# bbw7561135/Compton2d

Hardware: AMD Instinct MI355X
Metric: photon-packet-steps/sec (whole node) at 1/2/4/8 GPUs; % HBM roofline (higher is better)
Workload: dtype f64

## Files before the change

### compton2d_amd/csrc/c2d_device.hpp

```cpp
#ifndef C2D_DEVICE_HPP
#define C2D_DEVICE_HPP

#include <stdint.h>
#include "../../include/compton2d.h"

namespace c2d {

#define C2D_IDX_BUCKETS 2048
struct Geo {
  double z[C2D_MAXZONE + 1];
  double r[C2D_MAXZONE + 1];
  double E_ph[C2D_N_VOL + 1];
  double E_field[C2D_NPHFIELD + 1];
  double hu[C2D_NPHOMAX + 2];
  double Elcmin[C2D_NPHLCMAX + 1];
  double Elcmax[C2D_NPHLCMAX + 1];
  double mu[C2D_NMUMAX + 1];
  int16_t eph_start[C2D_IDX_BUCKETS];
  int16_t efl_start[C2D_IDX_BUCKETS];
  int32_t eph_k0, efl_k0;
};
constexpr int GEO_DOUBLES = (int)(sizeof(Geo) / sizeof(double));

struct SpecDev {
// ... 155 lines not shown
  const double* f_nt;
  const double* Pnt;
  const double* n_e;
  const double* vfrac;
  const double* ewsv;
  const int64_t* vol_prefix;
  const int64_t* surf_prefix;
  const double* surf_ew;
  const double* surf_tbb;
  const int32_t* surf_spec;
  const double* tbbl;
  const SpecDev* spectra;
  int32_t n_spectra, nslot;
  const double* comtab;
  double comtab_du_inv;
  double egg_min;
  CensusSoA cin, cout;
  int64_t n_cin, cap_cout;
  uint32_t cens_chunk;
  unsigned long long* n_cout;
  const int32_t* clist;
  const int32_t* pool;
  const unsigned long long* pool_n;
  unsigned long long* pool_head;
  int32_t* out_list;
  unsigned long long* n_out;
  int32_t* relist;
  unsigned long long* n_relist;
  unsigned long long* relist_head;
  int64_t* cstate;
  double* ev;
  int64_t cap_ev;
  unsigned long long* n_ev_sh;
  int64_t cap_ev_sh;
  int64_t cap_q;
  PktSoA pk;
  int64_t cap_pk;
  int64_t n_cens_items, n_vol_items, n_surf_items;
  int64_t vol_cens_base;
  int64_t n_vol_global, n_surf_global;
  double* T;
  double* nf_rep;
  TallyOff off;
  unsigned long long* cnt;
  int32_t* err;
  int32_t lds_cells;
  int32_t evq_cap;
  unsigned long long* prof;
  const uint16_t* cdf_guide;
  int32_t cr_sent;
  const double* refl_E;
  const double* refl_P;
  const double* refl_W;
  double* refl_out;
};
#define C2D_CDF_GUIDE 256

#define C2D_KN_CAP_DEFAULT 32
#define C2D_SC_K1_DEFAULT 16
struct GenArgs {
  const ScatRec* q2_in;
  const ScatRec* q3_in;
  ScatRec* q2_out;
  ScatRec* q3_out;
  unsigned long long* n2_out;
  unsigned long long* n3_out;
  unsigned long long* n_pk;
  unsigned long long* work_counter;
  unsigned long long* work_sh;
  unsigned long long* n_hard;
  int64_t* hard;
  int64_t item_begin, item_end;
  int64_t n_items;
  int64_t n2_in, n3_in;
  int32_t gen;
  int32_t kn_cap;
  int32_t sc_k1;
};

enum : int32_t {
  VZ_TEA = 0, VZ_TNA, VZ_NE, VZ_B, VZ_FPAIR, VZ_ZSURF, VZ_VOL, VZ_EP, VZ_LMIN, VZ_N = 12
};
enum : int32_t { VO_B = 0, VO_ESY, VO_ECY, VO_ETH, VO_ETOT, VO_N = 8 };
struct VemParams {
  const double* zin;
  const double* f_nt;
  const double* gnt;
  const double* E_ph;
  const double* mcd;
  double dE, pow3_15, dt;
  double* kappa;
  double* eps_tot;
  double* eps_th;
  double* zout;
};

enum : int32_t {
  FZ_VOL = 0, FZ_TEA, FZ_TNA, FZ_NE, FZ_B, FZ_ELSY, FZ_ECENS, FZ_ECOLD, FZ_TURB, FZ_FPAIR,
  FZ_PNTH, FZ_N = 16
};
enum : int32_t { FO_TE = 0, FO_NE, FO_GMIN, FO_GMAX, FO_AMXWL, FO_PNTH, FO_DIAG = 8, FO_N = 16 };
enum : int32_t { FPERR_STEPS = 1, FPERR_GUARD = 2, FPERR_NF_IN = 4, FPERR_NF_OUT = 8 };

#define C2D_FP_MCD_N 16384
#define C2D_FPF_MT_Q 1024
#define C2D_FPF_MT_LO (-17)
#define C2D_FPF_MT_HI 3
#define C2D_FPF_MT_N ((C2D_FPF_MT_HI - C2D_FPF_MT_LO) * C2D_FPF_MT_Q + 1)
#define C2D_FPF_MT_K 7
#define C2D_FPF_MT_W (4 + 2 * C2D_FPF_MT_K + 24)

struct FpParams {
  int32_t nz, nr, pick_sw, inj_switch, inj_dis, g2var_switch, cf_sentinel, pair_sw;
  double time, dt, df_implicit, df_T, r_esc, r_acc;
  double r_flare, z_flare, t_flare, sigma_r, sigma_z, sigma_t, flare_amp;
  double inj_g1, inj_g2, inj_p, inj_t, inj_L, pick_rate, inj_gg, inj_sigma, inj_v;
  const Geo* geo;
  const double* gnt;
  const double* FT;
  const double* mcd;
  const double* zin;
  const double* f_in;
  const double* P_in;
  const double* nf;
  const double* ecens;
  double* f_out;
  double* P_out;
  double* zout;
  int32_t* err;
  unsigned long long* gb_key;
  double* gb_val;
  uint32_t gb_mask;
  const int32_t* zorder;
  int32_t* zq;
  int32_t ncell;
  const double* mom;
  int32_t mt_glob;
  int32_t probe;
};

struct ObsDev {
  double gam_bulk, rmax, t_offset;
  int32_t mode, n_t, n_mu, n_e;
  const double* t0; const double* t1;
  const double* mu0; const double* mu1;
  const double* E0; const double* E1;
  double* F;
  double* F2;
  double* cnt;
  int32_t lds_rows;
  int32_t sorted_t, sorted_mu, sorted_e;
};

constexpr int OBS_SET_MAX = 8;
constexpr int OBS_SET_LDS = 64 * 1024;
constexpr int OBS_SET_LDS_STATIC = 1024;

struct ObsSetMember {
  double gam_bulk, rmax, t_offset;
  double* F; double* F2; double* cnt;
  int32_t mode, n_t, n_mu, n_e;
  int32_t lds_rows;
  int32_t sorted_t, sorted_mu, sorted_e;
  int32_t edge_off, hist_off;
};

struct ObsSetDev {
  const double* edges;
  int32_t n, n_edges, n_hist;
  ObsSetMember m[OBS_SET_MAX];
};

}

#endif
```

### compton2d_amd/csrc/capi.cpp

```cpp
#include <hip/hip_runtime.h>
#include <rccl/rccl.h>

#include <algorithm>
#include <cfloat>
#include <cmath>
#include <cstdarg>
#include <cstdio>
#include <cstring>
#include <string>
#include <vector>

#include "../../include/compton2d.h"
#include "c2d_device.hpp"
#include "c2d_math.h"
#include "c2d_rng.h"
#include "pspt_host.h"
#include "plcm_host.h"
#include "reflect_host.h"
#include "c2d_censfmt.h"
#include "c2d_censtext.hpp"
#include "c2d_evparse.hpp"
#include "c2d_evtext.hpp"

using namespace c2d;
// ... 141 lines not shown
  int64_t last_compact_moved = 0;
  c2d_tally_layout L;
  Geo* geo = nullptr;
  double *gnt = nullptr, *kappa_cur = nullptr, *kappa_prev = nullptr, *eps_tot = nullptr,
         *eps_th = nullptr, *f_nt = nullptr, *Pnt = nullptr, *n_e = nullptr, *vfrac = nullptr,
         *ewsv = nullptr, *surf_ew = nullptr, *surf_tbb = nullptr, *tbbl = nullptr;
  int64_t *vol_prefix = nullptr, *surf_prefix = nullptr;
  int32_t* surf_spec = nullptr;
  SpecDev* spectra = nullptr;
  std::vector<double*> spec_bufs;
  int n_spectra = 0;
  double* comtab = nullptr;
  double* comS = nullptr;
  DevCensus cens[2];
  int cur = 0;
  int64_t n_census = 0;
  double* ev = nullptr;
  int64_t n_ev = 0;
  int64_t ev_cnt[C2D_EV_SHARDS] = {};
  bool ev_stepped = false;
  c2d_evt_writer* evt = nullptr;
  c2d_evt_times evt_times = {};
  c2d_evt_reader* evr = nullptr;
  c2d_evr_times evr_times = {};
  c2d_cens_file* cfile = nullptr;
  c2d_cens_times cens_times = {};
  unsigned long long* cens_bad = nullptr;
  hipEvent_t cens_ev[2] = {nullptr, nullptr};
  hipStream_t obs_stream = nullptr;
  hipEvent_t ev_obs_src = nullptr, ev_obs_a = nullptr, ev_obs_b = nullptr;
  bool obs_inflight = false;
  int64_t ev_cap_sh = 0;
  ScatRec *q2[2] = {nullptr, nullptr}, *q3[2] = {nullptr, nullptr};
  DevPk pk;
  double* T = nullptr;
  double* T_own = nullptr;
  double* nf_rep = nullptr;
  unsigned long long* ctl = nullptr;
  int32_t* derr = nullptr;
  KParams* dP = nullptr;
  KParams P;
  bool have_step = false;
  bool have_electrons = false;
  bool have_vem = false;
  int32_t* mono_flag = nullptr;
  double* refl_tab = nullptr;
  double* refl_out = nullptr;
  double* refl_red = nullptr;
  bool refl_stepped = false;
  ncclComm_t comm = nullptr;
  int comm_rank = 0, comm_world = 1;
  int64_t n_vol_global = 0, n_surf_global = 0;
  int eps_linear = 0;
  uint16_t* cdf_guide = nullptr;
  bool cdf_guide_on = false;
  std::vector<double> h_stage;
  double last_g0_ms = 0.0, last_all_ms = 0.0;
  float last_src_ms = 0.f;
  unsigned long long last_prof[C2D_TR_PROF_WORDS] = {};
  int64_t last_g0_steps = 0;
  double egg_min = 0.0;
  int64_t last_g0_paths = 0, last_all_paths = 0;
  int last_launches = 0;
  bool fp_ready = false;
  c2d_fp_config fpc;
  double *fp_FT = nullptr, *fp_mcd = nullptr, *fp_zin = nullptr, *fp_fin = nullptr, *fp_Pin = nullptr,
         *fp_nf = nullptr, *fp_fout = nullptr, *fp_Pout = nullptr, *fp_zout = nullptr;
  int32_t* fp_err = nullptr;
  unsigned long long* fp_gb_key = nullptr;
  double* fp_gb_val = nullptr;
  int32_t fp_mode = C2D_FP_EXACT;
  unsigned long long* fpf_gb_key = nullptr;
  double* fpf_gb_val = nullptr;
  FpParams* fp_dP = nullptr;
  int32_t* fpf_zq = nullptr;
  double* fpf_mom = nullptr;
  std::vector<int32_t> fpf_order;
  bool fpf_ordered = false;
  bool fp_auto_known = false, fp_auto_exact = false;
  int32_t last_fp_mode = -1;
  float last_fp_ms = 0.f;
  int last_fp_waves = 0;
  double *vem_zin = nullptr, *vem_fnt = nullptr, *vem_eph = nullptr, *vem_kap = nullptr,
         *vem_et = nullptr, *vem_eh = nullptr, *vem_zout = nullptr;
  float last_vem_ms = 0.f;
  bool obs_ready = false;
  ObsDev obs;
  double *obs_edges = nullptr, *obs_hist = nullptr, *obs_ev = nullptr;
  double* pspt_red = nullptr;
  c2d_pspt_deck pspt;
  bool pspt_on = false;
  int64_t obs_ev_cap = 0;
  int obs_wg_per_cu = 1;
  double obs_ms = 0.0;
  ObsSetDev oset = {};
  std::vector<ObsSetHost> oset_h;
  double* oset_edges = nullptr;
  bool oset_started = false;
  bool obs_inflight_set = false;
  int oset_wg_per_cu = 1;
  int32_t oset_launches = 0;
  double oset_ms = 0.0;
};

static int fail(c2d_ctx* c, int code, const char* fmt, ...) {
  char buf[512];
  va_list ap;
  va_start(ap, fmt);
  vsnprintf(buf, sizeof buf, fmt, ap);
  va_end(ap);
  if (c) c->err = buf;
  return code;
}

#define HIPCHK(c, x)                                                                   \
  do {                                                                                 \
    hipError_t e_ = (x);                                                               \
    if (e_ != hipSuccess)                                                              \
      return fail((c), C2D_E_HIP, "%s:%d %s: %s", __FILE__, __LINE__, #x,              \
                  hipGetErrorString(e_));                                              \
  } while (0)

template <class T>
static hipError_t dalloc(T** p, size_t n) {
  if (n == 0) n = 1;
  return hipMalloc((void**)p, n * sizeof(T));
}

extern "C" const char* c2d_version(void) { return "compton2d_amd 0.1.0 (gfx950)"; }

extern "C" const char* c2d_last_error(c2d_ctx* ctx) { return ctx ? ctx->err.c_str() : "null context"; }

static __host__ __device__ int grid_bin_host(const double* E, int n, double x) {
  int lo = 1, hi = n;
  while (lo < hi) {
    const int mid = (lo + hi) >> 1;
    if (x < E[mid + 1]) hi = mid;
    else lo = mid + 1;
  }
  return lo;
}
static void build_lookup(const double* E, int n, int16_t* start, int32_t* k0) {
  uint64_t u;
  std::memcpy(&u, &E[1], sizeof u);
  *k0 = (int32_t)(u >> 48);
  for (int b = 0; b < C2D_IDX_BUCKETS; b++) {
    const uint64_t k = (uint64_t)(*k0 + b);
    double x = 0.0;
    if (k < 0x7ff0) {
      const uint64_t v = k << 48;
      std::memcpy(&x, &v, sizeof x);
      start[b] = (int16_t)grid_bin_host(E, n, x);
    } else {
      start[b] = (int16_t)(b > 0 ? start[b - 1] : 1);
    }
  }
}

extern "C" int c2d_init(const c2d_config* cfg, c2d_ctx** out) {
  if (!cfg || !out) return C2D_E_ARG;
  *out = nullptr;
  if (cfg->nz < 1 || cfg->nr < 1 || cfg->nz > C2D_MAXZONE || cfg->nr > C2D_MAXZONE)
    return C2D_E_ARG;
  if (cfg->nphtotal < 1 || cfg->nphtotal > C2D_NPHOMAX || cfg->nph_lc < 0 ||
      cfg->nph_lc > C2D_NPHLCMAX || cfg->nmu < 1 || cfg->nmu > C2D_NMUMAX)
    return C2D_E_ARG;
  if (cfg->cr_sent < 0 || cfg->cr_sent > 4) return C2D_E_ARG;
// ... 139 lines not shown
  {
    auto aocc = cfg->comtot_mode == C2D_COMTOT_TABLE ? c2d_aux_occupancy_fast : c2d_aux_occupancy_exact;
    int bs = 0, bc = 0;
    orc = aocc(0, &bs);
    if (!orc) orc = aocc(1, &bc);
    if (orc) return fail(c, C2D_E_HIP, "occupancy query: %s", hipGetErrorString((hipError_t)orc));
    c->src_grid = c->n_cu * std::max(1, bs);
    c->sc_grid = c->n_cu * std::max(1, bc);
  }
  {
    const int64_t ccap = std::max<int64_t>(cfg->census_capacity, 1);
    c->n_ws = (int64_t)std::max(c->bundle_grid, c->max_grid) * (C2D_TR_BLOCK / 64);
    HIPCHK(c, dalloc(&c->cstate, 2 * (size_t)c->n_ws));
    HIPCHK(c, hipMemset(c->cstate, 0xff, 2 * sizeof(int64_t) * c->n_ws));
    c->chunked = cfg->census_inplace ? 1 : 0;
    if (c->chunked) {
      c->cens_chunk = C2D_CCHUNK;
      int64_t slack = 4 * c->n_ws + 64;
      if (const char* e = getenv("C2D_CHUNK_SLACK")) slack = std::max<long long>(0, atoll(e));
      c->nchunks = (ccap + C2D_CCHUNK - 1) / C2D_CCHUNK + (ccap / 16 + C2D_CCHUNK - 1) / C2D_CCHUNK + slack;
      c->cens_phys = c->nchunks * C2D_CCHUNK;
      for (int b = 0; b < 2; b++) HIPCHK(c, dalloc(&c->clist[b], (size_t)c->nchunks));
      HIPCHK(c, dalloc(&c->pool, (size_t)c->nchunks));
      HIPCHK(c, dalloc(&c->out_list, (size_t)c->nchunks));
      HIPCHK(c, dalloc(&c->relist, (size_t)c->nchunks));
      HIPCHK(c, dalloc(&c->cflag, (size_t)c->nchunks));
      HIPCHK(c, dalloc(&c->part_id, (size_t)c->n_ws));
      HIPCHK(c, dalloc(&c->part_off, (size_t)c->n_ws + 1));
    } else {
      int64_t ch = 1024;
      while (ch > 64 && ch * c->n_ws * 8 > ccap) ch >>= 1;
      c->cens_chunk = (uint32_t)ch;
      c->cens_phys = ccap + c->n_ws * ch + 64;
      c->cscan_cap = std::min<int64_t>(int64_t(1) << 27, std::max<int64_t>(int64_t(1) << 16, ccap / 16));
      if (const char* e = getenv("C2D_COMPACT_LIST")) c->cscan_cap = std::max<long long>(1, atoll(e));
      HIPCHK(c, dalloc(&c->cscan, 2 * (size_t)c->cscan_cap));
    }
    for (int b = 0; b < (c->chunked ? 1 : 2); b++) {
      for (int f = 0; f < 3; f++) HIPCHK(c, dalloc(&c->cens[b].d[f], (size_t)c->cens_phys));
      HIPCHK(c, dalloc(&c->cens[b].tg, (size_t)c->cens_phys));
    }
  }
  HIPCHK(c, hipStreamSynchronize(c->stream));
  return C2D_OK;
}

extern "C" void c2d_finalize(c2d_ctx* c) {
  if (!c) return;
  (void)hipSetDevice(c->cfg.device);
  if (c->stream) (void)hipStreamSynchronize(c->stream);
  if (c->obs_stream) (void)hipStreamSynchronize(c->obs_stream);
  if (c->mono_flag) (void)hipFree(c->mono_flag);
  c2d_evtext_free(c->evt);
  c2d_evparse_free(c->evr);
  c2d_censtext_free(c->cfile);
  if (c->cens_bad) (void)hipFree(c->cens_bad);
  for (hipEvent_t e : c->cens_ev)
    if (e) (void)hipEventDestroy(e);
  if (c->comm) (void)ncclCommDestroy(c->comm);
  void* ptrs[] = {c->geo, c->gnt, c->kappa_cur, c->kappa_prev, c->eps_tot, c->eps_th, c->f_nt,
                  c->Pnt, c->n_e, c->vfrac, c->ewsv, c->surf_ew, c->surf_tbb, c->tbbl,
                  c->vol_prefix, c->surf_prefix, c->surf_spec, c->spectra, c->comtab, c->comS,
                  c->ev, c->q2[0], c->q2[1], c->q3[0], c->q3[1], c->T_own, c->nf_rep, c->ctl, c->derr, c->dP,
                  c->cscan, c->ctile_cnt, c->ctile_off, c->ctile_flag, c->cstate, c->clist[0], c->clist[1],
                  c->pool, c->out_list, c->relist, c->cflag, c->part_id, c->part_off, c->tmp_rec};
  for (void* p : ptrs)
    if (p) (void)hipFree(p);
  for (int b = 0; b < 2; b++) {
    for (int f = 0; f < 3; f++)
      if (c->cens[b].d[f]) (void)hipFree(c->cens[b].d[f]);
    if (c->cens[b].tg) (void)hipFree(c->cens[b].tg);
  }
  for (double* p : c->spec_bufs) (void)hipFree(p);
  void* rptrs[] = {c->refl_tab, c->refl_out, c->refl_red};
  for (void* p : rptrs)
    if (p) (void)hipFree(p);
  void* optrs[] = {c->obs_edges, c->obs_hist, c->obs_ev, c->pspt_red, c->cdf_guide, c->oset_edges};
  for (void* p : optrs)
    if (p) (void)hipFree(p);
  for (ObsSetHost& m : c->oset_h) {
    if (m.hist) (void)hipFree(m.hist);
    if (m.red) (void)hipFree(m.red);
  }
  void* vptrs[] = {c->vem_zin, c->vem_fnt, c->vem_eph, c->vem_kap, c->vem_et, c->vem_eh, c->vem_zout};
  for (void* q : vptrs)
    if (q) (void)hipFree(q);
  void* fptrs[] = {c->fp_FT, c->fp_mcd, c->fp_zin, c->fp_fin, c->fp_Pin, c->fp_nf, c->fp_fout, c->fp_Pout,
                   c->fp_zout, c->fp_err, c->fp_gb_key, c->fp_gb_val, c->fpf_gb_key, c->fpf_gb_val,
                   c->fp_dP, c->fpf_zq, c->fpf_mom};
  for (void* p : fptrs)
    if (p) (void)hipFree(p);
  c->pk.release();
  if (c->ev_g0a) (void)hipEventDestroy(c->ev_g0a);
  if (c->ev_g0b) (void)hipEventDestroy(c->ev_g0b);
  if (c->ev_g0t) (void)hipEventDestroy(c->ev_g0t);
  if (c->ev_end) (void)hipEventDestroy(c->ev_end);
  if (c->obs_stream) (void)hipStreamSynchronize(c->obs_stream);
  if (c->ev_obs_src) (void)hipEventDestroy(c->ev_obs_src);
  if (c->ev_obs_a) (void)hipEventDestroy(c->ev_obs_a);
  if (c->ev_obs_b) (void)hipEventDestroy(c->ev_obs_b);
  if (c->obs_stream) (void)hipStreamDestroy(c->obs_stream);
  if (c->stream) (void)hipStreamDestroy(c->stream);
  delete c;
}

static void gather3(const c2d_ctx* c, const c2d_array3& a, int n, double* out) {
  for (int j = 0; j < c->nz; j++)
    for (int k = 0; k < c->nr; k++) {
      double* o = out + (size_t)(j * c->nr + k) * n;
      if (!a.data) {
        std::fill(o, o + n, 0.0);
        continue;
      }
      const double* base = a.data + j * a.s_j + k * a.s_k;
      if (a.s_i == 1)
        memcpy(o, base, sizeof(double) * n);
      else
        for (int i = 0; i < n; i++) o[i] = base[i * a.s_i];
    }
}
static double at2(const c2d_array2& a, int j, int k) {
  return a.data ? a.data[j * a.s_j + k * a.s_k] : 0.0;
}

extern "C" int c2d_set_clock(c2d_ctx* c, int32_t ncycle, double time, double dt) {
  if (!c) return C2D_E_ARG;
  c->P.ncycle = ncycle;
  c->P.time = time;
  c->P.dt = dt;
  c->P.cdt = 2.9979245620e10 * dt;
  c->P.cens_wlim = c->cfg.trk_variant == C2D_TRK_2012_11 ? 1.0 : 0.99999999;
  c->P.step_key = c2d_step_key(c->cfg.seed, ncycle);
  return C2D_OK;
}

__global__ void __launch_bounds__(256) c2d_check_monotone(const double* __restrict__ a, int rows, int n,
                                                          int32_t* __restrict__ flag) {
  for (int64_t t = blockIdx.x * (int64_t)blockDim.x + threadIdx.x; t < (int64_t)rows * n;
       t += (int64_t)gridDim.x * blockDim.x) {
    const int i = (int)(t % n);
    if (i > 0 && !(a[t] >= a[t - 1])) atomicOr(flag, 1);
  }
}

__global__ void __launch_bounds__(256) c2d_check_finite(const double* __restrict__ a, int64_t n, int32_t bit,
                                                        int32_t* __restrict__ flag) {
  bool bad = false;
  for (int64_t t = blockIdx.x * (int64_t)blockDim.x + threadIdx.x; t < n; t += (int64_t)gridDim.x * blockDim.x)
    bad |= !(fabs(a[t]) <= DBL_MAX);
  if (bad) atomicOr(flag, bit);
}

static void check_finite(c2d_ctx* c, const double* a, int64_t n, int32_t bit, int32_t* flag, hipStream_t st) {
  if (n <= 0) return;
  const int grid = (int)std::max<int64_t>(1, std::min<int64_t>((n + 255) / 256, (int64_t)c->n_cu * 4));
  hipLaunchKernelGGL(c2d_check_finite, dim3(grid), dim3(256), 0, st, a, n, bit, flag);
}

static bool all_finite(const double* a, size_t n) {
  for (size_t i = 0; i < n; i++)
    if (!std::isfinite(a[i])) return false;
  return true;
}

__global__ void __launch_bounds__(256) c2d_cdf_guide(const double* __restrict__ eps_tot,
                                                     const double* __restrict__ eps_th, int ncell, int n,
                                                     uint16_t* __restrict__ guide) {
// ... 1707 lines not shown
      const double* dg = zo + FO_DIAG;
      double* p;
      if ((p = m2(out->Te_new, j, k))) *p = zo[FO_TE];
      if (dg[C2D_FP_SKIPPED] == 0.0) {
        for (int i = 0; i < C2D_NUM_NT && !el_dev; i++) {
          out->f_nt.data[i * out->f_nt.s_i + j * out->f_nt.s_j + k * out->f_nt.s_k] =
              fout[(size_t)cell * C2D_NUM_NT + i];
          out->Pnt.data[i * out->Pnt.s_i + j * out->Pnt.s_j + k * out->Pnt.s_k] =
              pout[(size_t)cell * C2D_NUM_NT + i];
        }
        if ((p = m2(out->n_e, j, k))) *p = zo[FO_NE];
        if ((p = m2(out->gmin, j, k))) *p = zo[FO_GMIN];
        if ((p = m2(out->gmax, j, k))) *p = zo[FO_GMAX];
        if ((p = m2(out->amxwl, j, k))) *p = zo[FO_AMXWL];
        if ((p = m2(out->p_nth, j, k))) *p = zo[FO_PNTH];
        E_old = E_old + dg[C2D_FP_E_OLD];
        E_new = E_new + dg[C2D_FP_E_NEW];
        hr = hr + dg[C2D_FP_HR];
        hr_st = hr_st + dg[C2D_FP_HR_ST];
        if (dg[C2D_FP_DELTA_T] > dT_max) dT_max = dg[C2D_FP_DELTA_T];
      }
      if ((p = m2(out->tea, j, k)) && a2(in->tna, j, k, 0.0) > 1.) {
        double t = zo[FO_TE];
        t = (1.0e3 < t) ? 1.0e3 : t;
        t = (5.0 > t) ? 5.0 : t;
        *p = t;
      }
      if (out->zone_diag)
        memcpy(out->zone_diag + (size_t)cell * C2D_FP_NDIAG, dg, sizeof(double) * C2D_FP_NDIAG);
    }
  out->E_tot_old = E_old;
  out->E_tot_new = E_new;
  out->hr_total = hr;
  out->hr_st_total = hr_st;
  out->dT_max = dT_max;
  return C2D_OK;
}

extern "C" int c2d_electron_state(c2d_ctx* c, c2d_marray3 f_nt, c2d_marray3 Pnt) {
  if (!c) return C2D_E_ARG;
  if (!c->have_electrons) return fail(c, C2D_E_STATE, "c2d_electron_state: no electron state yet");
  HIPCHK(c, hipSetDevice(c->cfg.device));
  const size_t nnt = (size_t)c->ncell * C2D_NUM_NT;
  std::vector<double> h(nnt);
  const c2d_marray3* views[2] = {&f_nt, &Pnt};
  const double* src[2] = {c->f_nt, c->Pnt};
  for (int v = 0; v < 2; v++) {
    const c2d_marray3& m = *views[v];
    if (!m.data) continue;
    HIPCHK(c, hipMemcpy(h.data(), src[v], nnt * sizeof(double), hipMemcpyDeviceToHost));
    for (int j = 0; j < c->nz; j++)
      for (int k = 0; k < c->nr; k++)
        for (int i = 0; i < C2D_NUM_NT; i++)
          m.data[i * m.s_i + j * m.s_j + k * m.s_k] = h[((size_t)j * c->nr + k) * C2D_NUM_NT + i];
  }
  return C2D_OK;
}

extern "C" int c2d_last_fp_ms(c2d_ctx* c, double* ms) {
  if (!c || !ms) return C2D_E_ARG;
  *ms = c->last_fp_ms;
  return C2D_OK;
}

extern "C" int c2d_volume_em(c2d_ctx* c, const c2d_vem_in* in, c2d_vem_out* out) {
  if (!c || !in || !out) return C2D_E_ARG;
  if (!in->tea.data || !in->tna.data || !in->n_e.data || !in->B_field.data || !in->f_pair.data ||
      !in->zsurf.data || !in->vol.data)
    return fail(c, C2D_E_ARG, "c2d_volume_em: missing input array");
  const bool el_dev = !in->f_nt.data;
  if (el_dev && !c->have_electrons)
    return fail(c, C2D_E_STATE, "c2d_volume_em: f_nt NULL but no electron state on the device");
  HIPCHK(c, hipSetDevice(c->cfg.device));
  const int nz = c->nz, nr = c->nr;
  const size_t nc = (size_t)c->ncell;
  if (!c->vem_zin) {
    HIPCHK(c, dalloc(&c->vem_zin, nc * VZ_N));
    HIPCHK(c, dalloc(&c->vem_fnt, nc * C2D_NUM_NT));
    HIPCHK(c, dalloc(&c->vem_eph, (size_t)C2D_N_VOL));
    HIPCHK(c, dalloc(&c->vem_kap, nc * C2D_N_VOL));
    HIPCHK(c, dalloc(&c->vem_et, nc * C2D_N_VOL));
    HIPCHK(c, dalloc(&c->vem_eh, nc * C2D_N_VOL));
    HIPCHK(c, dalloc(&c->vem_zout, nc * VO_N));
  }
  if (int rc = ensure_mcd(c)) return rc;
  const double dE = c2d_exp(c2d_log(1.0e20) / (double)C2D_N_VOL);
  std::vector<double> eph(C2D_N_VOL);
  double E = 1.0e-10 / dE;
  for (int i = 0; i < C2D_N_VOL; i++) {
    E = E * dE;
    eph[i] = E;
  }
  std::vector<double> zin(nc * VZ_N, 0.0), fnt(nc * C2D_NUM_NT);
  for (int j = 0; j < nz; j++)
    for (int k = 0; k < nr; k++) {
      const size_t cell = (size_t)j * nr + k;
      double* z = &zin[cell * VZ_N];
      z[VZ_TEA] = at2(in->tea, j, k);
      z[VZ_TNA] = at2(in->tna, j, k);
      z[VZ_NE] = at2(in->n_e, j, k);
      z[VZ_B] = at2(in->B_field, j, k);
      z[VZ_FPAIR] = at2(in->f_pair, j, k);
      if (c->cfg.pair_switch == 1 && !(z[VZ_FPAIR] < 1.0e-10))
        return fail(c, C2D_E_ARG,
                    "volume_em: pair annihilation (pair_switch=1, f_pair=%g in zone (%d,%d)) needs "
                    "a positron population; positrons are inert here (H6)", z[VZ_FPAIR], j + 1, k + 1);
      z[VZ_ZSURF] = at2(in->zsurf, j, k);
      z[VZ_VOL] = at2(in->vol, j, k);
      z[VZ_EP] = in->ep_switch.data ? (double)in->ep_switch.data[j * in->ep_switch.s_j + k * in->ep_switch.s_k] : 0.0;
      const double dz = (j == 0) ? c->cfg.z[0] : c->cfg.z[j] - c->cfg.z[j - 1];
      const double drr = (k == 0) ? c->cfg.r[0] - c->cfg.rmin : c->cfg.r[k] - c->cfg.r[k - 1];
      z[VZ_LMIN] = (dz < drr) ? dz : drr;
      for (int i = 0; i < C2D_NUM_NT && !el_dev; i++)
        fnt[cell * C2D_NUM_NT + i] = in->f_nt.data[i * in->f_nt.s_i + j * in->f_nt.s_j + k * in->f_nt.s_k];
    }
  if (!all_finite(zin.data(), zin.size()) || !all_finite(fnt.data(), el_dev ? 0 : fnt.size()))
    return fail(c, C2D_E_NONFINITE, "c2d_volume_em: NaN/Inf in the zone inputs or f_nt");
  c->have_vem = false;
  const hipStream_t st = c->stream;
  HIPCHK(c, hipMemcpyAsync(c->vem_zin, zin.data(), zin.size() * sizeof(double), hipMemcpyHostToDevice, st));
  if (!el_dev)
    HIPCHK(c, hipMemcpyAsync(c->vem_fnt, fnt.data(), fnt.size() * sizeof(double), hipMemcpyHostToDevice, st));
  HIPCHK(c, hipMemcpyAsync(c->vem_eph, eph.data(), eph.size() * sizeof(double), hipMemcpyHostToDevice, st));
  VemParams P;
  P.zin = c->vem_zin; P.f_nt = el_dev ? c->f_nt : c->vem_fnt; P.gnt = c->gnt; P.E_ph = c->vem_eph; P.mcd = c->fp_mcd;
  P.dE = dE; P.pow3_15 = c2d_pow(3.0, 1.5); P.dt = in->dt;
  P.kappa = c->vem_kap; P.eps_tot = c->vem_et; P.eps_th = c->vem_eh; P.zout = c->vem_zout;
  HIPCHK(c, hipEventRecord(c->ev_g0a, st));
  int rc = c2d_launch_vem(&P, (int)nc, st);
  if (rc) return fail(c, C2D_E_HIP, "vem launch: %s", hipGetErrorString((hipError_t)rc));
  HIPCHK(c, hipEventRecord(c->ev_g0b, st));
  if (!c->mono_flag) HIPCHK(c, dalloc(&c->mono_flag, 1));
  HIPCHK(c, hipMemsetAsync(c->mono_flag, 0, sizeof(int32_t), st));
  if (el_dev) check_finite(c, c->f_nt, (int64_t)nc * C2D_NUM_NT, 1, c->mono_flag, st);
  check_finite(c, c->vem_kap, (int64_t)nc * C2D_N_VOL, 2, c->mono_flag, st);
  check_finite(c, c->vem_et, (int64_t)nc * C2D_N_VOL, 2, c->mono_flag, st);
  check_finite(c, c->vem_eh, (int64_t)nc * C2D_N_VOL, 2, c->mono_flag, st);
  HIPCHK(c, hipGetLastError());
  int32_t vflag = 0;
  HIPCHK(c, hipMemcpyAsync(&vflag, c->mono_flag, sizeof vflag, hipMemcpyDeviceToHost, st));
  std::vector<double> kap(out->kappa_tot.data ? nc * C2D_N_VOL : 0),
      et(out->eps_tot.data ? nc * C2D_N_VOL : 0), eh(out->eps_th.data ? nc * C2D_N_VOL : 0), zo(nc * VO_N);
  if (!kap.empty())
    HIPCHK(c, hipMemcpyAsync(kap.data(), c->vem_kap, kap.size() * sizeof(double), hipMemcpyDeviceToHost, st));
  if (!et.empty())
    HIPCHK(c, hipMemcpyAsync(et.data(), c->vem_et, et.size() * sizeof(double), hipMemcpyDeviceToHost, st));
  if (!eh.empty())
    HIPCHK(c, hipMemcpyAsync(eh.data(), c->vem_eh, eh.size() * sizeof(double), hipMemcpyDeviceToHost, st));
  HIPCHK(c, hipMemcpyAsync(zo.data(), c->vem_zout, zo.size() * sizeof(double), hipMemcpyDeviceToHost, st));
  HIPCHK(c, hipStreamSynchronize(st));
  (void)hipEventElapsedTime(&c->last_vem_ms, c->ev_g0a, c->ev_g0b);
  if (vflag & 1) return fail(c, C2D_E_NONFINITE, "c2d_volume_em: NaN/Inf in the device f_nt");
  bool zo_ok = true;
  for (size_t cell = 0; cell < nc; cell++) zo_ok = zo_ok && all_finite(&zo[cell * VO_N], VO_ETOT + 1);
  if ((vflag & 2) || !zo_ok)
    return fail(c, C2D_E_NONFINITE, "c2d_volume_em: NaN/Inf in the emission/absorption tables or "
                "Eloss outputs (volume2d.f:343-390)");
  c->have_vem = true;
  if (out->E_ph) std::copy(eph.begin(), eph.end(), out->E_ph);
  auto put3 = [&](c2d_marray3& m, const std::vector<double>& v, size_t cell, int j, int k) {
    if (!m.data) return;
    for (int i = 0; i < C2D_N_VOL; i++)
      m.data[i * m.s_i + j * m.s_j + k * m.s_k] = v[cell * C2D_N_VOL + i];
  };
  auto put2 = [&](c2d_marray2& m, int j, int k, double v) {
    if (m.data) m.data[j * m.s_j + k * m.s_k] = v;
  };
  for (int j = 0; j < nz; j++)
    for (int k = 0; k < nr; k++) {
      const size_t cell = (size_t)j * nr + k;
      put3(out->kappa_tot, kap, cell, j, k);
      put3(out->eps_tot, et, cell, j, k);
      put3(out->eps_th, eh, cell, j, k);
      const double* o = &zo[cell * VO_N];
      put2(out->B_field, j, k, o[VO_B]);
      put2(out->Eloss_sy, j, k, o[VO_ESY]);
      put2(out->Eloss_cy, j, k, o[VO_ECY]);
      put2(out->Eloss_th, j, k, o[VO_ETH]);
      put2(out->Eloss_tot, j, k, o[VO_ETOT]);
    }
  return C2D_OK;
}

extern "C" int c2d_last_vem_ms(c2d_ctx* c, double* ms) {
  if (!c || !ms) return C2D_E_ARG;
  *ms = c->last_vem_ms;
  return C2D_OK;
}

static int obs_settle(c2d_ctx* c);

extern "C" int c2d_obs_begin(c2d_ctx* c, const c2d_obs_bins* b) {
  if (!c || !b) return C2D_E_ARG;
  if ((b->mode != C2D_OBS_SED && b->mode != C2D_OBS_LC) || b->n_t < 1 || b->n_t > C2D_OBS_MAX_T ||
      b->n_mu < 1 || b->n_mu > C2D_OBS_MAX_MU || b->n_e < 1 || b->n_e > C2D_OBS_MAX_E ||
      !b->t0 || !b->t1 || !b->mu0 || !b->mu1 || !b->E0 || !b->E1 || !(b->gam_bulk >= 1.0))
    return fail(c, C2D_E_ARG, "c2d_obs_begin: bad binning");
  if (b->mode == C2D_OBS_SED && b->n_mu != 1)
    return fail(c, C2D_E_ARG, "c2d_obs_begin: the SED mode has one angular window");
  c->pspt_on = false;
  c->obs_ready = false;
  HIPCHK(c, hipSetDevice(c->cfg.device));
  { const int rc = obs_settle(c); if (rc) return rc; }
  if (c->obs_edges) (void)hipFree(c->obs_edges);
  if (c->obs_hist) (void)hipFree(c->obs_hist);
  c->obs_edges = c->obs_hist = nullptr;
  const int ne = 2 * (b->n_t + b->n_mu + b->n_e);
  std::vector<double> h;
  h.reserve(ne);
  h.insert(h.end(), b->t0, b->t0 + b->n_t);
// ... 909 lines not shown
```

### compton2d_amd/csrc/vem.hip

```cpp
#include <hip/hip_runtime.h>
#include <stdint.h>

#include "c2d_device.hpp"
#include "c2d_math.h"
#include "c2d_wave.hpp"

namespace c2d {
namespace {

using namespace wave;
constexpr int VEM_BLOCK = 448;
constexpr int NT = C2D_NUM_NT;
constexpr int NV = C2D_N_VOL;
constexpr double PI_REF = 3.1415926536;
constexpr double C_LIGHT = 2.9979245620e10;

__device__ __forceinline__ double expk13(double t) {
  const double c1 = F32(0.35502805), c2 = F32(0.25881940);
  if (t <= 1.0) {
    double z3 = 1.5 * t;
    const double zs = c2d_pow(z3, 0.3333333333333333);
    const double z = zs * zs;
    z3 = z3 * z3;
    const double f1 = 1.0 + z3 / 6.0 * (1.0 + z3 / 30.0 * (1.0 + z3 / 56.0));
    const double f2 = z * (1.0 + z3 / 12.0 * (1.0 + z3 / 42.0 * (1.0 + z3 / 90.0)));
    return c2d_exp_bf(t) * PI_REF * 1.7320508 / zs * (c1 * f1 - c2 * f2);
  }
  const double z = 1.0 / (72.0 * t);
  const double poly = 1.0 - 5.0 * z * (1.0 - 38.5 * z);
  return __builtin_sqrt(0.5 * PI_REF / t) * poly / (1.0 + 1.0 / (1.0 + 58.0 * t * t));
}

__device__ __forceinline__ double expk43(double t) {
  if (t <= 1.0) {
    const double poly = 1.0 + t * (0.9757317 - 7.6790616e-2 * t);
    return 0.44648975 * c2d_pow(2.0 / t, 1.333333333) * poly;
  }
  const double z = 1.0 / (72.0 * t);
  const double poly = 1.0 + 55.0 * z * (1.0 - 8.5 * z);
  return __builtin_sqrt(0.5 * PI_REF / t) * poly * (1.0 + 1.0 / (1.0 + 50.0 * t * t));
}

}

__global__ void __launch_bounds__(VEM_BLOCK) c2d_vem_kernel(const VemParams P) {
  __shared__ double s_gnt[NT], s_f[NT], s_q[NT], s_gamp[NT], s_facg[NT], s_dg[NT];
  __shared__ double s_cP[NV], s_cC[NV], s_cT[NV], s_P[NV], s_Pth[NV];
  __shared__ double s_sc[8];
  __shared__ double s_mcd[4 * FPB];
  const int cell = blockIdx.x;
  const int tid = threadIdx.x, lane = tid & 63, wv = tid >> 6;
  const double* zin = P.zin + (int64_t)cell * VZ_N;
  const double tea = zin[VZ_TEA], ne = zin[VZ_NE];
  for (int i = tid; i < NT; i += VEM_BLOCK) {
    s_gnt[i] = P.gnt[i];
    s_f[i] = P.f_nt[(int64_t)cell * NT + i];
  }
  __syncthreads();
  if (wv == 0) {
    long long guard = 0;
    double B = zin[VZ_B];
    const int ep = (int)zin[VZ_EP];
    if (ep == 1 || ep == 2) {
      const double Th = (ep == 1) ? 1.957e-3 * tea : 1.066e-6 * zin[VZ_TNA];
      double uB;
      if (Th < 1.0e-2) {
        uB = 1.5 * Th + 7.5 * (Th * Th);
      } else {
        double K2b, K3b;
        mcdonald23_w(1.0 / Th, lane, P.mcd, K2b, K3b, guard, s_mcd);
        uB = K3b / K2b - Th - 1.0;
      }
      if (ep == 1)
        uB = uB * ne * 8.176e-7 * (1. + 2.0 * zin[VZ_FPAIR]);
      else
        uB = uB * ne * 1.5e-3;
      B = __builtin_sqrt(2.513e1 * uB);
    }
    const double Theta = tea / 5.11e2;
    double K2 = 0.0, K2m = 0.0, K3m = 0.0;
    const bool big = !(Theta < F32(0.2)) || !(Theta < 2.0e-1);
    if (big) mcdonald23_w(1. / Theta, lane, P.mcd, K2m, K3m, guard, s_mcd);
    if (Theta < 2.0e-1)
      K2 = 1.2533 * __builtin_sqrt(Theta) *
           (1. + 1.875 * Theta + 8.2031e-1 * (Theta * Theta) - 2.03e-1 * (Theta * Theta * Theta)) /
           c2d_exp_bf(Theta);
    else
      K2 = K2m;
    double g_av;
    if (Theta < F32(0.2)) {
      g_av = (1. + F32(4.375) * Theta + F32(7.383) * (Theta * Theta) +
              F32(3.384) * (Theta * Theta * Theta)) /
                 (1. + F32(1.875) * Theta + F32(.8203) * (Theta * Theta)) -
             Theta;
    } else {
      g_av = K3m / K2m - Theta;
    }
    if (g_av < 1.0) g_av = 1.0;
    const double gamma_R = 2.1e-3 * __builtin_sqrt(ne) / (B * __builtin_sqrt(g_av));
    const double y = gamma_R / g_av;
    const double f_rz = (y < 1.0e2) ? c2d_exp_bf(-y) : 0.;
    const double s1 = seq_sum(0.0, 0, NT - 2, lane, [&](int i) {
      const double g1 = s_gnt[i] + 1.0;
      return (g1 * g1 - 1.0) * s_f[i] * (s_gnt[i + 1] - s_gnt[i]);
    });
    if (lane == 0) {
      s_sc[0] = B; s_sc[1] = K2; s_sc[2] = f_rz; s_sc[7] = s1;
    }
  }
  __syncthreads();
  const double B = s_sc[0], K2 = s_sc[1], f_rz = s_sc[2];
  const double em = 9.109e-28, ee = 4.803e-10, sigmaT = 6.6524616e-25;
  const double nu_b = ee * B / (2 * PI_REF * em * C_LIGHT);
  for (int i = tid; i < NT; i += VEM_BLOCK) {
    const double g0 = s_gnt[i] + 1.0;
    const double gp = g0 * __builtin_sqrt(g0 * g0 - 1.0);
    s_gamp[i] = gp;
    s_q[i] = s_f[i] / gp;
    s_facg[i] = 3.0 * (g0 * g0) * nu_b;
    s_dg[i] = (i < NT - 1) ? s_gnt[i + 1] - s_gnt[i] : 0.0;
  }
  __syncthreads();
  if (tid < NV) {
    const int i = tid;
    const double Ub = (B * B) / (8.0 * PI_REF);
    const double face = P.pow3_15 * sigmaT * C_LIGHT * Ub / (PI_REF * nu_b);
    const double dE = P.dE, E = P.E_ph[i];
    const double Theta = tea / 5.11e2;
    const double kappa_C = 6.65e-25 * ne;
    const double nu_c = 2.8e6 * B, nu_min = 5.0 * nu_c, nu_p = 9.0e3 * __builtin_sqrt(ne);
    const double nu = 2.41487e17 * E;
    double j_sy = 0., kappa_sy = 0., j_cy = 0.;
    if (!(nu <= nu_p)) {
      double sum = 0., sum_k = 0.;
      for (int i2 = 0; i2 < NT - 1; i2++) {
        const double tt = nu / s_facg[i2];
        double es = 0.0;
        if (tt < 1.0e4) {
          const double eq43 = expk43(tt), eq13 = expk13(tt);
          const double ff = tt * tt * (eq43 * eq13 - F32(0.6) * tt * (eq43 - eq13) * (eq43 + eq13));
          es = face * ff * c2d_exp_bf(-2.0 * tt);
        }
        const double sd = s_f[i2] * es;
        const double sd_k = s_gamp[i2] * es;
        sum = sum + s_dg[i2] * sd;
        sum_k = sum_k + (s_q[i2] - s_q[i2 + 1]) * sd_k;
      }
      j_sy = sum * ne / (4.0 * PI_REF);
      kappa_sy = sum_k * ne / (8.0 * PI_REF * em * (nu * nu));
      if (kappa_sy < 0.) kappa_sy = -1.0 * kappa_sy;
      double f_m = 1.0;
      for (int m = 1; m <= 5; m++) {
        const double mm = (double)m;
        f_m = f_m / (4. * mm);
        const double nu_m = mm * nu_c;
        const double E_m = 4.14e-18 * nu_m;
        const double D_m = 7.07e-1 * Theta * E_m;
        const double q = (E - E_m) / D_m;
        const double x = q * q;
        if (x < 50.) {
          const double f_cy = f_rz * c2d_exp_bf(-x) * ne * (B * B) * c2d_pow(Theta, mm - 1.5) *
                              (mm + 1.0) * f_m * c2d_pow(mm, 2.0 * mm + 1.0);
          j_cy = j_cy + 8.46e-14 * f_cy * (E * E) / (E_m * E_m * E_m);
        }
      }
      if (nu > nu_min) {
        const double v = nu / (nu_c * (Theta * Theta));
        const double y = 4.5 * v;
        if (y < 1.0e6)
          j_cy = j_cy + 4.652e-12 * ne * nu /
                            (K2 * c2d_pow(v, 1.6666667e-1) * c2d_exp_bf(c2d_pow(y, 3.33333e-1)));
      }
    }
    P.kappa[(int64_t)cell * NV + i] = kappa_sy;
    const double lm = zin[VZ_LMIN];
    const double thr = (1.0 / lm > 1.0e1 * kappa_C) ? 1.0 / lm : 1.0e1 * kappa_C;
    double cP = 0.0, cC = 0.0, cT = 0.0;
    if (kappa_sy < thr) {
      cP = j_sy * E * (dE - 1.0);
      cC = j_cy * E * (dE - 1.0);
    } else {
      const double x = E / tea;
      const double tau_tot = kappa_sy * lm;
      double j_th = (x < 1.0e2) ? 1.47e-47 * (nu * nu * nu) / (c2d_exp_bf(x) - 1.0) : 1.0e-50;
      if (tau_tot < 5.0e1) j_th = j_th * (1.0 - c2d_exp_bf(-tau_tot));
      cT = j_th * E * (dE - 1.0);
    }
    s_cP[i] = cP; s_cC[i] = cC; s_cT[i] = cT;
  }
  __syncthreads();
  if (wv == 0) {
    double aP = 0.0, aT = 0.0, aC = 0.0;
    for (int c0 = 0; c0 < NV; c0 += FPB) {
      const int i = c0 + lane;
      const double vP = (i < NV) ? s_cP[i] : 0.0, vT = (i < NV) ? s_cT[i] : 0.0;
      const double vC = (i < NV) ? s_cC[i] : 0.0;
      const int mn = (NV - c0) < FPB ? (NV - c0) : FPB;
      double mP = 0.0, mT = 0.0;
      for (int m = 0; m < mn; m++) {
        aP = aP + rl(vP, m);
        aT = aT + rl(vT, m);
        aC = aC + rl(vC, m);
        if (lane == m) { mP = aP; mT = aT; }
      }
      if (i < NV) { s_P[i] = mP; s_Pth[i] = mT; }
    }
    if (lane == 0) {
      s_sc[3] = aP; s_sc[4] = aT; s_sc[5] = aC;
    }
  }
  __syncthreads();
  if (tid < NV) {
    const double P_sum = s_sc[3], sum_th = s_sc[4];
    P.eps_tot[(int64_t)cell * NV + tid] = (P_sum > 1.0e-50) ? s_P[tid] / P_sum : 0.;
    P.eps_th[(int64_t)cell * NV + tid] = (sum_th > 1.0e-50) ? s_Pth[tid] / sum_th : 0.;
  }
  if (tid == 0) {
    const double vol = zin[VZ_VOL], zs = zin[VZ_ZSURF], dt = P.dt;
    double* o = P.zout + (int64_t)cell * VO_N;
    const double esy = 1.058e-15 * ne * dt * (B * B) * s_sc[7] * vol;
    o[VO_B] = B;
    o[VO_ESY] = esy;
    o[VO_ECY] = dt * vol * s_sc[5];
    o[VO_ETH] = dt * zs * s_sc[4];
    o[VO_ETOT] = esy;
  }
}

}

extern "C" int c2d_launch_vem(const c2d::VemParams* P, int ncell, hipStream_t stream) {
  if (ncell <= 0) return 0;
  hipLaunchKernelGGL(c2d::c2d_vem_kernel, dim3(ncell), dim3(c2d::VEM_BLOCK), 0, stream, *P);
  return (int)hipGetLastError();
}
```

Measured before the change: 291.7 billion.

## Split volume-emission kernel into per-cell, per-energy-chunk, and closing passes

```diff
diff --git a/compton2d_amd/csrc/c2d_device.hpp b/compton2d_amd/csrc/c2d_device.hpp
--- a/compton2d_amd/csrc/c2d_device.hpp
+++ b/compton2d_amd/csrc/c2d_device.hpp
@@ -261,6 +261,7 @@
   VZ_TEA = 0, VZ_TNA, VZ_NE, VZ_B, VZ_FPAIR, VZ_ZSURF, VZ_VOL, VZ_EP, VZ_LMIN, VZ_N = 12
 };
 enum : int32_t { VO_B = 0, VO_ESY, VO_ECY, VO_ETH, VO_ETOT, VO_N = 8 };
+enum : int32_t { VEM_SC_N = 4 };
 struct VemParams {
   const double* zin;
   const double* f_nt;
@@ -272,6 +273,8 @@
   double* eps_tot;
   double* eps_th;
   double* zout;
+  double* cell_sc;
+  double* contrib_cy;
 };
 
 enum : int32_t {
diff --git a/compton2d_amd/csrc/capi.cpp b/compton2d_amd/csrc/capi.cpp
--- a/compton2d_amd/csrc/capi.cpp
+++ b/compton2d_amd/csrc/capi.cpp
@@ -247,7 +247,7 @@
   float last_fp_ms = 0.f;
   int last_fp_waves = 0;
   double *vem_zin = nullptr, *vem_fnt = nullptr, *vem_eph = nullptr, *vem_kap = nullptr,
-         *vem_et = nullptr, *vem_eh = nullptr, *vem_zout = nullptr;
+         *vem_et = nullptr, *vem_eh = nullptr, *vem_zout = nullptr, *vem_sc = nullptr, *vem_cy = nullptr;
   float last_vem_ms = 0.f;
   bool obs_ready = false;
   ObsDev obs;
@@ -553,7 +553,8 @@
     if (m.hist) (void)hipFree(m.hist);
     if (m.red) (void)hipFree(m.red);
   }
-  void* vptrs[] = {c->vem_zin, c->vem_fnt, c->vem_eph, c->vem_kap, c->vem_et, c->vem_eh, c->vem_zout};
+  void* vptrs[] = {c->vem_zin, c->vem_fnt, c->vem_eph, c->vem_kap, c->vem_et, c->vem_eh, c->vem_zout,
+                   c->vem_sc, c->vem_cy};
   for (void* q : vptrs)
     if (q) (void)hipFree(q);
   void* fptrs[] = {c->fp_FT, c->fp_mcd, c->fp_zin, c->fp_fin, c->fp_Pin, c->fp_nf, c->fp_fout, c->fp_Pout,
@@ -2427,6 +2428,8 @@
     HIPCHK(c, dalloc(&c->vem_et, nc * C2D_N_VOL));
     HIPCHK(c, dalloc(&c->vem_eh, nc * C2D_N_VOL));
     HIPCHK(c, dalloc(&c->vem_zout, nc * VO_N));
+    HIPCHK(c, dalloc(&c->vem_sc, nc * VEM_SC_N));
+    HIPCHK(c, dalloc(&c->vem_cy, nc * C2D_N_VOL));
   }
   if (int rc = ensure_mcd(c)) return rc;
   const double dE = c2d_exp(c2d_log(1.0e20) / (double)C2D_N_VOL);
@@ -2471,6 +2474,7 @@
   P.zin = c->vem_zin; P.f_nt = el_dev ? c->f_nt : c->vem_fnt; P.gnt = c->gnt; P.E_ph = c->vem_eph; P.mcd = c->fp_mcd;
   P.dE = dE; P.pow3_15 = c2d_pow(3.0, 1.5); P.dt = in->dt;
   P.kappa = c->vem_kap; P.eps_tot = c->vem_et; P.eps_th = c->vem_eh; P.zout = c->vem_zout;
+  P.cell_sc = c->vem_sc; P.contrib_cy = c->vem_cy;
   HIPCHK(c, hipEventRecord(c->ev_g0a, st));
   int rc = c2d_launch_vem(&P, (int)nc, st);
   if (rc) return fail(c, C2D_E_HIP, "vem launch: %s", hipGetErrorString((hipError_t)rc));
diff --git a/compton2d_amd/csrc/vem.hip b/compton2d_amd/csrc/vem.hip
--- a/compton2d_amd/csrc/vem.hip
+++ b/compton2d_amd/csrc/vem.hip
@@ -9,7 +9,6 @@
 namespace {
 
 using namespace wave;
-constexpr int VEM_BLOCK = 448;
 constexpr int NT = C2D_NUM_NT;
 constexpr int NV = C2D_N_VOL;
 constexpr double PI_REF = 3.1415926536;
@@ -43,97 +42,110 @@
 
 }
 
-__global__ void __launch_bounds__(VEM_BLOCK) c2d_vem_kernel(const VemParams P) {
-  __shared__ double s_gnt[NT], s_f[NT], s_q[NT], s_gamp[NT], s_facg[NT], s_dg[NT];
-  __shared__ double s_cP[NV], s_cC[NV], s_cT[NV], s_P[NV], s_Pth[NV];
-  __shared__ double s_sc[8];
+constexpr int VEM_EPB = 8;
+constexpr int VEM_LPE = 32;
+constexpr int VEM_TBLOCK = VEM_EPB * VEM_LPE;
+static_assert(NV % VEM_EPB == 0, "whole workgroups of energies");
+static_assert(VEM_TBLOCK >= 128 && VEM_TBLOCK >= NT, "two waves; one pass over the electron grid");
+
+__global__ void __launch_bounds__(FPB) c2d_vem_cell(const VemParams P) {
+  __shared__ double s_gnt[NT], s_f[NT];
   __shared__ double s_mcd[4 * FPB];
   const int cell = blockIdx.x;
-  const int tid = threadIdx.x, lane = tid & 63, wv = tid >> 6;
+  const int lane = threadIdx.x;
   const double* zin = P.zin + (int64_t)cell * VZ_N;
   const double tea = zin[VZ_TEA], ne = zin[VZ_NE];
-  for (int i = tid; i < NT; i += VEM_BLOCK) {
+  for (int i = lane; i < NT; i += FPB) {
     s_gnt[i] = P.gnt[i];
     s_f[i] = P.f_nt[(int64_t)cell * NT + i];
   }
   __syncthreads();
-  if (wv == 0) {
-    long long guard = 0;
-    double B = zin[VZ_B];
-    const int ep = (int)zin[VZ_EP];
-    if (ep == 1 || ep == 2) {
-      const double Th = (ep == 1) ? 1.957e-3 * tea : 1.066e-6 * zin[VZ_TNA];
-      double uB;
-      if (Th < 1.0e-2) {
-        uB = 1.5 * Th + 7.5 * (Th * Th);
-      } else {
-        double K2b, K3b;
-        mcdonald23_w(1.0 / Th, lane, P.mcd, K2b, K3b, guard, s_mcd);
-        uB = K3b / K2b - Th - 1.0;
-      }
-      if (ep == 1)
-        uB = uB * ne * 8.176e-7 * (1. + 2.0 * zin[VZ_FPAIR]);
-      else
-        uB = uB * ne * 1.5e-3;
-      B = __builtin_sqrt(2.513e1 * uB);
-    }
-    const double Theta = tea / 5.11e2;
-    double K2 = 0.0, K2m = 0.0, K3m = 0.0;
-    const bool big = !(Theta < F32(0.2)) || !(Theta < 2.0e-1);
-    if (big) mcdonald23_w(1. / Theta, lane, P.mcd, K2m, K3m, guard, s_mcd);
-    if (Theta < 2.0e-1)
-      K2 = 1.2533 * __builtin_sqrt(Theta) *
-           (1. + 1.875 * Theta + 8.2031e-1 * (Theta * Theta) - 2.03e-1 * (Theta * Theta * Theta)) /
-           c2d_exp_bf(Theta);
+  long long guard = 0;
+  double B = zin[VZ_B];
+  const int ep = (int)zin[VZ_EP];
+  if (ep == 1 || ep == 2) {
+    const double Th = (ep == 1) ? 1.957e-3 * tea : 1.066e-6 * zin[VZ_TNA];
+    double uB;
+    if (Th < 1.0e-2) {
+      uB = 1.5 * Th + 7.5 * (Th * Th);
+    } else {
+      double K2b, K3b;
+      mcdonald23_w(1.0 / Th, lane, P.mcd, K2b, K3b, guard, s_mcd);
+      uB = K3b / K2b - Th - 1.0;
+    }
+    if (ep == 1)
+      uB = uB * ne * 8.176e-7 * (1. + 2.0 * zin[VZ_FPAIR]);
     else
-      K2 = K2m;
-    double g_av;
-    if (Theta < F32(0.2)) {
-      g_av = (1. + F32(4.375) * Theta + F32(7.383) * (Theta * Theta) +
-              F32(3.384) * (Theta * Theta * Theta)) /
-                 (1. + F32(1.875) * Theta + F32(.8203) * (Theta * Theta)) -
-             Theta;
-    } else {
-      g_av = K3m / K2m - Theta;
-    }
-    if (g_av < 1.0) g_av = 1.0;
-    const double gamma_R = 2.1e-3 * __builtin_sqrt(ne) / (B * __builtin_sqrt(g_av));
-    const double y = gamma_R / g_av;
-    const double f_rz = (y < 1.0e2) ? c2d_exp_bf(-y) : 0.;
-    const double s1 = seq_sum(0.0, 0, NT - 2, lane, [&](int i) {
-      const double g1 = s_gnt[i] + 1.0;
-      return (g1 * g1 - 1.0) * s_f[i] * (s_gnt[i + 1] - s_gnt[i]);
-    });
-    if (lane == 0) {
-      s_sc[0] = B; s_sc[1] = K2; s_sc[2] = f_rz; s_sc[7] = s1;
-    }
-  }
-  __syncthreads();
-  const double B = s_sc[0], K2 = s_sc[1], f_rz = s_sc[2];
+      uB = uB * ne * 1.5e-3;
+    B = __builtin_sqrt(2.513e1 * uB);
+  }
+  const double Theta = tea / 5.11e2;
+  double K2 = 0.0, K2m = 0.0, K3m = 0.0;
+  const bool big = !(Theta < F32(0.2)) || !(Theta < 2.0e-1);
+  if (big) mcdonald23_w(1. / Theta, lane, P.mcd, K2m, K3m, guard, s_mcd);
+  if (Theta < 2.0e-1)
+    K2 = 1.2533 * __builtin_sqrt(Theta) *
+         (1. + 1.875 * Theta + 8.2031e-1 * (Theta * Theta) - 2.03e-1 * (Theta * Theta * Theta)) /
+         c2d_exp_bf(Theta);
+  else
+    K2 = K2m;
+  double g_av;
+  if (Theta < F32(0.2)) {
+    g_av = (1. + F32(4.375) * Theta + F32(7.383) * (Theta * Theta) +
+            F32(3.384) * (Theta * Theta * Theta)) /
+               (1. + F32(1.875) * Theta + F32(.8203) * (Theta * Theta)) -
+           Theta;
+  } else {
+    g_av = K3m / K2m - Theta;
+  }
+  if (g_av < 1.0) g_av = 1.0;
+  const double gamma_R = 2.1e-3 * __builtin_sqrt(ne) / (B * __builtin_sqrt(g_av));
+  const double y = gamma_R / g_av;
+  const double f_rz = (y < 1.0e2) ? c2d_exp_bf(-y) : 0.;
+  const double s1 = seq_sum(0.0, 0, NT - 2, lane, [&](int i) {
+    const double g1 = s_gnt[i] + 1.0;
+    return (g1 * g1 - 1.0) * s_f[i] * (s_gnt[i + 1] - s_gnt[i]);
+  });
+  if (lane == 0) {
+    double* sc = P.cell_sc + (int64_t)cell * VEM_SC_N;
+    sc[0] = B; sc[1] = K2; sc[2] = f_rz; sc[3] = s1;
+  }
+}
+
+__global__ void __launch_bounds__(VEM_TBLOCK) c2d_vem_terms(const VemParams P) {
+  __shared__ double s_f[NT], s_q[NT], s_gamp[NT], s_facg[NT], s_dg[NT];
+  __shared__ double s_t[VEM_EPB][NT], s_tk[VEM_EPB][NT];
+  __shared__ double s_sk[VEM_EPB], s_jcy[VEM_EPB];
+  constexpr int NCHUNK = NV / VEM_EPB;
+  const int cell = blockIdx.x / NCHUNK;
+  const int e0 = (blockIdx.x % NCHUNK) * VEM_EPB;
+  const int tid = threadIdx.x;
+  const double* zin = P.zin + (int64_t)cell * VZ_N;
+  const double* sc = P.cell_sc + (int64_t)cell * VEM_SC_N;
+  const double tea = zin[VZ_TEA], ne = zin[VZ_NE];
+  const double B = sc[0], K2 = sc[1], f_rz = sc[2];
   const double em = 9.109e-28, ee = 4.803e-10, sigmaT = 6.6524616e-25;
   const double nu_b = ee * B / (2 * PI_REF * em * C_LIGHT);
-  for (int i = tid; i < NT; i += VEM_BLOCK) {
-    const double g0 = s_gnt[i] + 1.0;
+  if (tid < NT) {
+    const int i = tid;
+    const double gn = P.gnt[i], f = P.f_nt[(int64_t)cell * NT + i];
+    const double g0 = gn + 1.0;
     const double gp = g0 * __builtin_sqrt(g0 * g0 - 1.0);
+    s_f[i] = f;
     s_gamp[i] = gp;
-    s_q[i] = s_f[i] / gp;
+    s_q[i] = f / gp;
     s_facg[i] = 3.0 * (g0 * g0) * nu_b;
-    s_dg[i] = (i < NT - 1) ? s_gnt[i + 1] - s_gnt[i] : 0.0;
-  }
-  __syncthreads();
-  if (tid < NV) {
-    const int i = tid;
-    const double Ub = (B * B) / (8.0 * PI_REF);
-    const double face = P.pow3_15 * sigmaT * C_LIGHT * Ub / (PI_REF * nu_b);
-    const double dE = P.dE, E = P.E_ph[i];
-    const double Theta = tea / 5.11e2;
-    const double kappa_C = 6.65e-25 * ne;
-    const double nu_c = 2.8e6 * B, nu_min = 5.0 * nu_c, nu_p = 9.0e3 * __builtin_sqrt(ne);
-    const double nu = 2.41487e17 * E;
-    double j_sy = 0., kappa_sy = 0., j_cy = 0.;
+    s_dg[i] = (i < NT - 1) ? P.gnt[i + 1] - gn : 0.0;
+  }
+  __syncthreads();
+  const double Ub = (B * B) / (8.0 * PI_REF);
+  const double face = P.pow3_15 * sigmaT * C_LIGHT * Ub / (PI_REF * nu_b);
+  const double nu_c = 2.8e6 * B, nu_min = 5.0 * nu_c, nu_p = 9.0e3 * __builtin_sqrt(ne);
+  {
+    const int el = tid / VEM_LPE, l = tid % VEM_LPE;
+    const double nu = 2.41487e17 * P.E_ph[e0 + el];
     if (!(nu <= nu_p)) {
-      double sum = 0., sum_k = 0.;
-      for (int i2 = 0; i2 < NT - 1; i2++) {
+      for (int i2 = l; i2 < NT - 1; i2 += VEM_LPE) {
         const double tt = nu / s_facg[i2];
         double es = 0.0;
         if (tt < 1.0e4) {
@@ -143,12 +155,27 @@
         }
         const double sd = s_f[i2] * es;
         const double sd_k = s_gamp[i2] * es;
-        sum = sum + s_dg[i2] * sd;
-        sum_k = sum_k + (s_q[i2] - s_q[i2 + 1]) * sd_k;
+        s_t[el][i2] = s_dg[i2] * sd;
+        s_tk[el][i2] = (s_q[i2] - s_q[i2 + 1]) * sd_k;
       }
-      j_sy = sum * ne / (4.0 * PI_REF);
-      kappa_sy = sum_k * ne / (8.0 * PI_REF * em * (nu * nu));
-      if (kappa_sy < 0.) kappa_sy = -1.0 * kappa_sy;
+    }
+  }
+  __syncthreads();
+  const int i = e0 + (tid & (VEM_EPB - 1));
+  const double E = P.E_ph[i];
+  const double nu = 2.41487e17 * E;
+  const double Theta = tea / 5.11e2;
+  const bool on = !(nu <= nu_p);
+  double sum = 0.;
+  if (tid < 2 * VEM_EPB) {
+    if (on) {
+      const double* t = tid < VEM_EPB ? s_t[tid] : s_tk[tid - VEM_EPB];
+      for (int i2 = 0; i2 < NT - 1; i2++) sum = sum + t[i2];
+    }
+    if (tid >= VEM_EPB) s_sk[tid - VEM_EPB] = sum;
+  } else if (tid >= FPB && tid < FPB + VEM_EPB) {
+    double j_cy = 0.;
+    if (on) {
       double f_m = 1.0;
       for (int m = 1; m <= 5; m++) {
         const double mm = (double)m;
@@ -172,6 +199,19 @@
                             (K2 * c2d_pow(v, 1.6666667e-1) * c2d_exp_bf(c2d_pow(y, 3.33333e-1)));
       }
     }
+    s_jcy[tid - FPB] = j_cy;
+  }
+  __syncthreads();
+  if (tid < VEM_EPB) {
+    const double dE = P.dE;
+    const double kappa_C = 6.65e-25 * ne;
+    double j_sy = 0., kappa_sy = 0.;
+    const double j_cy = s_jcy[tid];
+    if (on) {
+      j_sy = sum * ne / (4.0 * PI_REF);
+      kappa_sy = s_sk[tid] * ne / (8.0 * PI_REF * em * (nu * nu));
+      if (kappa_sy < 0.) kappa_sy = -1.0 * kappa_sy;
+    }
     P.kappa[(int64_t)cell * NV + i] = kappa_sy;
     const double lm = zin[VZ_LMIN];
     const double thr = (1.0 / lm > 1.0e1 * kappa_C) ? 1.0 / lm : 1.0e1 * kappa_C;
@@ -186,43 +226,55 @@
       if (tau_tot < 5.0e1) j_th = j_th * (1.0 - c2d_exp_bf(-tau_tot));
       cT = j_th * E * (dE - 1.0);
     }
-    s_cP[i] = cP; s_cC[i] = cC; s_cT[i] = cT;
-  }
-  __syncthreads();
-  if (wv == 0) {
-    double aP = 0.0, aT = 0.0, aC = 0.0;
-    for (int c0 = 0; c0 < NV; c0 += FPB) {
-      const int i = c0 + lane;
-      const double vP = (i < NV) ? s_cP[i] : 0.0, vT = (i < NV) ? s_cT[i] : 0.0;
-      const double vC = (i < NV) ? s_cC[i] : 0.0;
-      const int mn = (NV - c0) < FPB ? (NV - c0) : FPB;
-      double mP = 0.0, mT = 0.0;
-      for (int m = 0; m < mn; m++) {
-        aP = aP + rl(vP, m);
-        aT = aT + rl(vT, m);
-        aC = aC + rl(vC, m);
-        if (lane == m) { mP = aP; mT = aT; }
-      }
-      if (i < NV) { s_P[i] = mP; s_Pth[i] = mT; }
-    }
-    if (lane == 0) {
-      s_sc[3] = aP; s_sc[4] = aT; s_sc[5] = aC;
-    }
-  }
-  __syncthreads();
-  if (tid < NV) {
-    const double P_sum = s_sc[3], sum_th = s_sc[4];
-    P.eps_tot[(int64_t)cell * NV + tid] = (P_sum > 1.0e-50) ? s_P[tid] / P_sum : 0.;
-    P.eps_th[(int64_t)cell * NV + tid] = (sum_th > 1.0e-50) ? s_Pth[tid] / sum_th : 0.;
-  }
-  if (tid == 0) {
-    const double vol = zin[VZ_VOL], zs = zin[VZ_ZSURF], dt = P.dt;
+    P.eps_tot[(int64_t)cell * NV + i] = cP;
+    P.eps_th[(int64_t)cell * NV + i] = cT;
+    P.contrib_cy[(int64_t)cell * NV + i] = cC;
+  }
+}
+
+__global__ void __launch_bounds__(FPB) c2d_vem_close(const VemParams P) {
+  const int cell = blockIdx.x;
+  const int lane = threadIdx.x;
+  double* et = P.eps_tot + (int64_t)cell * NV;
+  double* eh = P.eps_th + (int64_t)cell * NV;
+  const double* cy = P.contrib_cy + (int64_t)cell * NV;
+  constexpr int NC = (NV + FPB - 1) / FPB;
+  double aP = 0.0, aT = 0.0, aC = 0.0;
+  double mP[NC], mT[NC];
+#pragma unroll
+  for (int c = 0; c < NC; c++) {
+    const int c0 = c * FPB;
+    const int i = c0 + lane;
+    const double vP = (i < NV) ? et[i] : 0.0, vT = (i < NV) ? eh[i] : 0.0;
+    const double vC = (i < NV) ? cy[i] : 0.0;
+    const int mn = (NV - c0) < FPB ? (NV - c0) : FPB;
+    mP[c] = 0.0; mT[c] = 0.0;
+    for (int m = 0; m < mn; m++) {
+      aP = aP + rl(vP, m);
+      aT = aT + rl(vT, m);
+      aC = aC + rl(vC, m);
+      if (lane == m) { mP[c] = aP; mT[c] = aT; }
+    }
+  }
+#pragma unroll
+  for (int c = 0; c < NC; c++) {
+    const int i = c * FPB + lane;
+    if (i < NV) {
+      et[i] = (aP > 1.0e-50) ? mP[c] / aP : 0.;
+      eh[i] = (aT > 1.0e-50) ? mT[c] / aT : 0.;
+    }
+  }
+  if (lane == 0) {
+    const double* zin = P.zin + (int64_t)cell * VZ_N;
+    const double* sc = P.cell_sc + (int64_t)cell * VEM_SC_N;
+    const double ne = zin[VZ_NE], vol = zin[VZ_VOL], zs = zin[VZ_ZSURF], dt = P.dt;
+    const double B = sc[0];
     double* o = P.zout + (int64_t)cell * VO_N;
-    const double esy = 1.058e-15 * ne * dt * (B * B) * s_sc[7] * vol;
+    const double esy = 1.058e-15 * ne * dt * (B * B) * sc[3] * vol;
     o[VO_B] = B;
     o[VO_ESY] = esy;
-    o[VO_ECY] = dt * vol * s_sc[5];
-    o[VO_ETH] = dt * zs * s_sc[4];
+    o[VO_ECY] = dt * vol * aC;
+    o[VO_ETH] = dt * zs * aT;
     o[VO_ETOT] = esy;
   }
 }
@@ -231,6 +283,9 @@
 
 extern "C" int c2d_launch_vem(const c2d::VemParams* P, int ncell, hipStream_t stream) {
   if (ncell <= 0) return 0;
-  hipLaunchKernelGGL(c2d::c2d_vem_kernel, dim3(ncell), dim3(c2d::VEM_BLOCK), 0, stream, *P);
+  hipLaunchKernelGGL(c2d::c2d_vem_cell, dim3(ncell), dim3(c2d::FPB), 0, stream, *P);
+  hipLaunchKernelGGL(c2d::c2d_vem_terms, dim3(ncell * (c2d::NV / c2d::VEM_EPB)), dim3(c2d::VEM_TBLOCK), 0,
+                     stream, *P);
+  hipLaunchKernelGGL(c2d::c2d_vem_close, dim3(ncell), dim3(c2d::FPB), 0, stream, *P);
   return (int)hipGetLastError();
 }
```

Measured after the change: 292.5 billion (median of 6 runs). About the same (+0.3%).
